# zachramsey/pm-rl

Measured on AMD Instinct MI355X. Metric: env-steps/sec (whole node) at 65k envs x 30 assets; reward MAE vs CPU ref, higher is better.
Workload: dtype f64

## Files before the change

pm-rl_amd/csrc/common.h:

```cpp
#pragma once
#include <hip/hip_runtime.h>

#include <math.h>
#include <stdint.h>

#include "../../include/pmenv.h"
#include "step_plan.h"

namespace pmenv_dev {

constexpr uint32_t kRelaySpin = 1024;

typedef float f4 __attribute__((ext_vector_type(4)));
typedef float f4u __attribute__((ext_vector_type(4), aligned(4)));

struct FastDiv {
    uint32_t mul, shift, d;
};

inline FastDiv make_fastdiv(uint32_t d) {
    FastDiv f;
    f.d = d;
    uint32_t s = 0;
    while ((1ull << s) < d) ++s;
// ... 37 lines not shown
    uint32_t halo_wgs, halo_block, halo_qtot;
    uint32_t halo_hs;
    const double* sv_in;
    const int32_t* sk_in;
    const float* sw_in;
    const float* slc_in;
    double* sv_out;
    int32_t* sk_out;
    float* sw_out;
    float* slc_out;
    const float* halo_in;
    float* halo_out;
    uint32_t per4;
    int32_t* seq;
    FastDiv div_wf, div_f, div_w, div_units;
};

struct HostIO {
    const float* close_in;
    float* chan;
    double* value_out;
    uint32_t* done;
    uint32_t seq;
};


__device__ __forceinline__ const float* env_bar(const StepParams& p, int b) {
    const size_t row = (size_t)p.N * (p.F - 1);
    if (!p.day) return p.bar + (size_t)b * row;
    const int32_t d = p.day[b];
// ... 89 lines not shown
```

pm-rl_amd/csrc/env_step.h:

```cpp
#pragma once
#include "common.h"

namespace pmenv_dev {

struct Scratch {
    double* wv;
    double* yv;
    float* wl;
    float* wp;
    float* bar;
    int* ints;
    int wp_off, bar_off;
};

__device__ __forceinline__ Scratch carve(float* lds, int tile_floats, int N, int F) {
    Scratch s;
    s.wv = reinterpret_cast<double*>(lds + tile_floats);
    s.yv = s.wv + N;
    s.wl = reinterpret_cast<float*>(s.yv + N);
    s.wp = s.wl + N;
    s.bar = s.wp + N;
    s.ints = reinterpret_cast<int*>(s.bar + N * (F - 1));
    s.wp_off = tile_floats + 4 * N + N;
    s.bar_off = s.wp_off + N;
// ... 809 lines not shown
    for (int e = 0; e < 4; ++e) {
        const int pos = sd.kk + e;
        const bool in_row = pos < WF;
        const bool lastday = in_row && pos >= WF - F;
        const bool is_w = in_row && f == F - 1;
        const float bsel = pick(sd.bar_nan, __int_as_float(0x7fc00000),
                                pick(f == 0, sd.xb.x, pick(f == 1, sd.xb.y, pick(f == 2, sd.xb.z, sd.xb.w))));
        const bool w_here = shift_w ? lastday : pos == slot_w;
        const float wv = pick(w_here, sd.xwp, pick(shift_w, sh[e], un[e]));
        v[e] = pick(is_w, wv, pick(lastday, bsel, sh[e]));
        f = f == F - 1 ? 0 : f + 1;
    }
    return f4{v[0], v[1], v[2], v[3]};
}

template <typename Side>
__device__ __forceinline__ f4 compose2(const StepParams& p, int kk, int32_t k, const float (&un)[4],
                                       const float (&sh)[4], Side side) {
    constexpr int F = 5;
    const int W = p.W, WF = W * F;
    const bool shift_w = !(p.ring_mode == PMENV_RING_STORAGE && k >= W - 1);
    const int f0 = kk - (int)fdiv((uint32_t)kk, p.div_f) * F;
    float o[4];
#pragma unroll
    for (int e = 0; e < 4; ++e) {
        const int f = f0 + e >= F ? f0 + e - F : f0 + e;
        o[e] = pick(!shift_w & (f == F - 1), un[e], sh[e]);
    }
    const int slot_w = (int)(((uint32_t)(1 + k) - fdiv((uint32_t)(1 + k), p.div_w) * (uint32_t)W) * F + (F - 1));
    if ((kk + 3 >= WF - F) | (!shift_w & ((uint32_t)(slot_w - kk) <= 3u))) {
        f4 xb;
        float xwp;
        side(xb, xwp);
#pragma unroll
        for (int e = 0; e < 4; ++e) {
            const int pos = kk + e;
            const int f = f0 + e >= F ? f0 + e - F : f0 + e;
            const bool in_row = pos < WF;
            const bool lastday = in_row & (pos >= WF - F);
            const float bsel = pick(f == 0, xb.x, pick(f == 1, xb.y, pick(f == 2, xb.z, xb.w)));
            o[e] = pick(lastday & (f < F - 1), bsel, o[e]);
            o[e] = pick((shift_w & lastday & (f == F - 1)) | (!shift_w & in_row & (pos == slot_w)), xwp, o[e]);
        }
    }
    return f4{o[0], o[1], o[2], o[3]};
}

template <int BLOCK, int POL>
__global__ __launch_bounds__(BLOCK) void advance_flat_kernel(StepParams p, uint32_t qtot) {
    constexpr int kAux = POL == 1 ? 2 : POL == 2 ? 3 : 0;
    const int lane = threadIdx.x & 63;
    const uint32_t wbase = __builtin_amdgcn_readfirstlane(blockIdx.x * BLOCK + (threadIdx.x & ~63u));
    if (wbase >= qtot) return;
    const uint32_t nwave = min(64u, qtot - wbase);
    const auto rs_src = make_rsrc(p.obs + (size_t)wbase * 4, nwave * 16u);
    const f4 own = buf_load4<kAux>(rs_src, (uint32_t)lane * 16u);
    const uint32_t qx = wbase + 64u;
// ... 72 lines not shown
            sd[v].xb = sh_side[wave][ri[v]];
            sd[v].xwp = reinterpret_cast<const float*>(&sh_side[wave][4])[ri[v]];
        }
        const f4 n1 = sh4[j + 1], n2 = sh4[j + 2];
        const float sh[4] = {n1.y, n1.z, n1.w, n2.x};
        const float un[4] = {own[v].x, own[v].y, own[v].z, own[v].w};
        if (ABL & 128) buf_store4<kAux>(rd, (uint32_t)j * 16u, f4{sh[0], sh[1], sh[2], sh[3]});
        else buf_store4<kAux>(rd, (uint32_t)j * 16u, flat_compose(p, sd[v], un, sh));
    }
}

template <int BLOCK, int V, int POL, bool OUT>
__device__ __forceinline__ void flat_wg_body_patch(StepParams& p, uint32_t qtot, f4* sh4) {
    constexpr int kAux = POL == 1 ? 2 : POL == 2 ? 3 : 0;
    constexpr int CPW = BLOCK * V, F = 5;
    __shared__ f4 sh_bar[BLOCK];
    __shared__ float sh_wp[BLOCK];
    __shared__ int32_t sh_kc[BLOCK];
    const int tid = threadIdx.x, lane = tid & 63, wave = tid >> 6;
    const uint32_t c0 = blockIdx.x * CPW;
    const uint32_t nblk = min((uint32_t)CPW, qtot - c0);
    const auto rs = make_rsrc(p.obs + (size_t)c0 * 4, nblk * 16u);
    f4 own[V];
#pragma unroll
    for (int v = 0; v < V; ++v) own[v] = buf_load4<kAux>(rs, (uint32_t)(64 * V * wave + 64 * v + lane) * 16u);
    const uint32_t nh = blockIdx.x + 1 < gridDim.x ? min(2u, qtot - c0 - nblk) : 0u;
    const float* hsrc = OUT ? p.obs + (size_t)(c0 + nblk) * 4 : p.halo + (size_t)blockIdx.x * 8;
    const f4 hal = buf_load4<0>(make_rsrc(hsrc, nh * 16u), tid < 2 ? (uint32_t)tid * 16u : 0xFFFFFFF0u);
    __builtin_amdgcn_sched_barrier(0);
    const int N = p.N, W = p.W, WF = W * F;
    const uint32_t per4 = (uint32_t)(N * WF) >> 2;
    const uint32_t b_lo = fdiv(c0, p.div_units);
    const uint32_t g_lo = b_lo * (uint32_t)N + fdiv(4u * (c0 - b_lo * per4), p.div_wf);
    const uint32_t ql = c0 + nblk - 1u;
    const uint32_t b_hi = fdiv(ql, p.div_units);
    const uint32_t g_hi = b_hi * (uint32_t)N + fdiv(4u * (ql - b_hi * per4) + 3u, p.div_wf);
    if ((uint32_t)tid <= g_hi - g_lo) {
        const uint32_t g = g_lo + (uint32_t)tid;
        const uint32_t b = g / (uint32_t)N, n = g - b * (uint32_t)N;
        const float* barb = env_bar(p, (int)b);
        const float nanv = __int_as_float(0x7fc00000);
        sh_bar[tid] = barb ? *reinterpret_cast<const f4*>(barb + (size_t)n * 4) : f4{nanv, nanv, nanv, nanv};
        sh_wp[tid] = p.w_new[g];
        sh_kc[tid] = p.k[b] - 1;
    }
#pragma unroll
    for (int v = 0; v < V; ++v) sh4[64 * V * wave + 64 * v + lane] = own[v];
    if (tid < 2) sh4[CPW + tid] = hal;
    __syncthreads();
    const auto rd = OUT ? make_rsrc(p.obs_out + (size_t)c0 * 4, nblk * 16u) : rs;
#pragma unroll
    for (int v = 0; v < V; ++v) {
        const int j = 64 * V * wave + 64 * v + lane;
        const uint32_t q = min(c0 + (uint32_t)j, qtot - 1u);
        const uint32_t b = fdiv(q, p.div_units);
        const uint32_t j0 = 4u * (q - b * per4);
        const uint32_t row = fdiv(j0, p.div_wf);
        const int kk = (int)(j0 - row * (uint32_t)WF);
        const int t = (int)(b * (uint32_t)N + row - g_lo);
        const f4 n1 = sh4[j + 1], n2 = sh4[j + 2];
        const float sh[4] = {n1.y, n1.z, n1.w, n2.x};
        const float un[4] = {own[v].x, own[v].y, own[v].z, own[v].w};
        const f4 o = compose2(p, kk, sh_kc[t], un, sh, [&](f4& xb, float& xwp) {
            xb = sh_bar[t];
            xwp = sh_wp[t];
        });
        buf_store4<kAux>(rd, (uint32_t)j * 16u, o);
    }
}

template <int BLOCK, int V, int POL, int ABL = 0>
__global__ __launch_bounds__(BLOCK) void advance_flat_inplace_kernel(StepParams p, uint32_t qtot) {
    __shared__ f4 sh4[BLOCK * V + 2];
    if constexpr (ABL == 0) flat_wg_body_patch<BLOCK, V, POL, false>(p, qtot, sh4);
    else flat_wg_body<BLOCK, V, POL, false, ABL>(p, qtot, sh4);
}

template <int BLOCK, int V, int POL>
__global__ __launch_bounds__(BLOCK) void advance_flat_inplace_perelem_kernel(StepParams p, uint32_t qtot) {
    __shared__ f4 sh4[BLOCK * V + 2];
    flat_wg_body<BLOCK, V, POL, false, 0>(p, qtot, sh4);
}
template <int BLOCK, int V, int POL>
// ... 700 lines not shown
```

pm-rl_amd/csrc/handle.h:

```cpp
#pragma once
#include <hip/hip_runtime.h>

#include <stdarg.h>
#include <stdio.h>
#include <stdlib.h>
#include <string.h>

#include "../../include/pmenv.h"
#include "common.h"
#include "step_plan.h"

struct pmenv : pmenv_host::StepPlan {
    pmenv_cfg cfg;
    int device;
    void* state;
    size_t state_bytes;
    bool owns_state;
    double* value;
    double* sa;
    double* sb;
    int32_t* k;
    float* ring;
    float* last_close;
    float* w_new;
// ... 71 lines not shown
    p.ret_mode = c.ret_mode; p.mu_max_iter = c.mu_max_iter;
    p.rows_per_tile = h->rows_per_tile;
    p.tile_floats = h->tile_floats;
    p.unit_rows = h->unit_rows;
    p.units_per_env = h->units_per_env;
    p.init_cash = c.init_cash; p.commission = c.commission; p.scale = c.reward_scale;
    p.rf = c.risk_free_rate; p.eta = c.sharpe_eta; p.mu_tol = c.mu_tol;
    p.value = h->value; p.k = h->k; p.ring = h->ring; p.last_close = h->last_close;
    p.w_new = h->w_new;
    p.sa = h->sa; p.sb = h->sb;
    p.nonfinite = h->nonfinite;
    p.div_wf = make_fastdiv((uint32_t)(c.window * c.features));
    p.div_f = make_fastdiv((uint32_t)c.features);
    p.div_w = make_fastdiv((uint32_t)c.window);
    p.div_units = make_fastdiv((uint32_t)(h->units_per_env > 0 ? h->units_per_env : 1));
    return p;
}

inline bool aligned4(const void* ptr) { return ((uintptr_t)ptr & 3u) == 0; }

inline int device_cus() {
    static const int cus = [] {
        int dev = 0, n = 0;
        if (hipGetDevice(&dev) != hipSuccess ||
            hipDeviceGetAttribute(&n, hipDeviceAttributeMultiprocessorCount, dev) != hipSuccess || n <= 0)
            n = 256;
        return n;
    }();
    return cus;
}
// ... 47 lines not shown
```

pm-rl_amd/csrc/step_flat.h:

```cpp
#pragma once
#include "scalar_vec.h"

namespace pmenv_dev {

__device__ __forceinline__ ScalarIn scalar_load_snap(const StepParams& p, int b, int lane) {
    const int N = p.N;
    const uint32_t nb = (uint32_t)N * 4u, off = (uint32_t)lane * 4u;
    ScalarIn in;
    in.k = p.sk_in[b];
    in.v_prev = p.sv_in[b];
    in.sa = p.sa[b];
    in.sb = p.sb[b];
    in.a = buf_load1(make_rsrc(p.action + (size_t)b * N, nb), off);
    in.wlf = buf_load1(make_rsrc(p.sw_in + (size_t)b * N, p.commission > 0.0 ? nb : 0u), off);
    in.pl = buf_load1(make_rsrc((p.prices ? p.prices : p.slc_in) + (size_t)b * N, nb), off);
    const float* barb = env_bar(p, b);
    in.bar = buf_load4(make_rsrc(barb ? barb : p.bar, barb ? nb * 4u : 0u), off * 4u);
    in.bar_ok = barb != nullptr;
    in.cn = 0.0f;
    return in;
}

template <int V>
struct FlatTile {
// ... 14 lines not shown
    t.ne = (int)(fdiv(t.c0 + t.nblk - 1u, p.div_units) - t.e_lo) + 1;
    if (wave < t.ne) t.sin = scalar_load_snap(p, (int)t.e_lo + wave, lane);
    __builtin_amdgcn_sched_barrier(0);
    const auto rs = make_rsrc(p.obs + (size_t)t.c0 * 4, t.nblk * 16u);
#pragma unroll
    for (int v = 0; v < V; ++v) t.own[v] = buf_load4<AUX>(rs, (uint32_t)(64 * V * wave + 64 * v + lane) * 16u);
    const uint32_t ntiles = (qtot + CPW - 1) / CPW;
    const uint32_t nh = tile + 1 < ntiles ? min(2u, qtot - t.c0 - t.nblk) : 0u;
    const float* hsrc = OUT ? p.obs + (size_t)(t.c0 + t.nblk) * 4 : p.halo_in + (size_t)tile * 8;
    t.hal = buf_load4<0>(make_rsrc(hsrc, nh * 16u), tid < 2 ? (uint32_t)tid * 16u : 0xFFFFFFF0u);
    __builtin_amdgcn_sched_barrier(0);
}

template <int BLOCK, int V, int AUX, bool OUT>
__device__ __forceinline__ void flat1_process(const StepParams& p, uint32_t qtot, uint32_t tile, const FlatTile<V>& t,
                                              f4* sh4, f4 (*sh_bar)[64], float (*sh_wp)[64], int32_t* sh_k) {
    constexpr int CPW = BLOCK * V, F = 5;
    const int tid = threadIdx.x, lane = tid & 63, wave = __builtin_amdgcn_readfirstlane(tid >> 6);
    const uint32_t per4 = p.per4;
    ScalarMid mid;
    if (wave < t.ne) {
        mid = scalar_core<64, true>(p, (int)t.e_lo + wave, lane, t.sin);
        sh_wp[wave][lane] = mid.wp;
        sh_bar[wave][lane] = t.sin.bar_ok ? t.sin.bar : f4{NAN, NAN, NAN, NAN};
        if (lane == 0) sh_k[wave] = mid.k;
    }
#pragma unroll
    for (int v = 0; v < V; ++v) sh4[64 * V * wave + 64 * v + lane] = t.own[v];
    if (tid < 2) sh4[CPW + tid] = t.hal;
    __syncthreads();
    const int WF = p.W * F;
    const auto rd = make_rsrc((OUT ? p.obs_out : p.obs) + (size_t)t.c0 * 4, t.nblk * 16u);
    const bool first_out = !OUT && tile > 0;
#pragma unroll
    for (int v = 0; v < V; ++v) {
        const int j = 64 * V * wave + 64 * v + lane;
        const uint32_t q = min(t.c0 + (uint32_t)j, qtot - 1u);
        const uint32_t e = fdiv(q, p.div_units);
        const int le = (int)(e - t.e_lo);
        const uint32_t j0 = 4u * (q - e * per4);
        const uint32_t row = fdiv(j0, p.div_wf);
        const int kk = (int)(j0 - row * (uint32_t)WF);
        const f4 n1 = sh4[j + 1], n2 = sh4[j + 2];
        const float sh[4] = {n1.y, n1.z, n1.w, n2.x};
        const float un[4] = {t.own[v].x, t.own[v].y, t.own[v].z, t.own[v].w};
        const f4 o = compose2(p, kk, sh_k[le], un, sh, [&](f4& xb, float& xwp) {
            xb = sh_bar[le][row];
            xwp = sh_wp[le][row];
        });
        buf_store4<AUX>(rd, (uint32_t)j * 16u, o);
        if (first_out && j < 2) reinterpret_cast<f4*>(p.halo_out)[2 * (tile - 1) + j] = o;
    }
    if (wave < t.ne) {
        const int b = (int)t.e_lo + wave;
        const bool owner = (uint64_t)b * per4 >= t.c0;
        scalar_tail<64, true>(p, b, lane, t.sin, mid, owner);
    }
}

template <bool OUT>
__device__ __forceinline__ void flat_seq_enter(StepParams& p) {
    if (!p.seq) return;
    const int c = __builtin_amdgcn_readfirstlane(p.seq[1]);
    if (c) {
        const double* v = p.sv_in; p.sv_in = p.sv_out; p.sv_out = const_cast<double*>(v);
        const int32_t* k = p.sk_in; p.sk_in = p.sk_out; p.sk_out = const_cast<int32_t*>(k);
        const float* w = p.sw_in; p.sw_in = p.sw_out; p.sw_out = const_cast<float*>(w);
// ... 2 lines not shown
    }
    if (blockIdx.x == 0 && threadIdx.x == 0) {
        const uint64_t hobs = OUT ? 0ull : (uint64_t)(uintptr_t)p.obs;
        p.seq[0] = 1 - c;
        p.seq[2] = 1;
        p.seq[4] = (int32_t)(uint32_t)hobs;
        p.seq[5] = (int32_t)(uint32_t)(hobs >> 32);
    }
}

template <int BLOCK, int V, int POL, bool OUT>
__global__ __launch_bounds__(BLOCK) __attribute__((amdgpu_num_sgpr(80))) void step_flat_kernel(StepParams p,
                                                                                              uint32_t qtot) {
    constexpr int CPW = BLOCK * V, WAVES = BLOCK / 64, AUX = POL == 1 ? 2 : 0;
    __shared__ f4 sh4[CPW + 2];
    __shared__ f4 sh_bar[WAVES][64];
    __shared__ float sh_wp[WAVES][64];
    __shared__ int32_t sh_k[WAVES];
    flat_seq_enter<OUT>(p);
    FlatTile<V> t;
    flat1_load<BLOCK, V, AUX, OUT>(p, qtot, blockIdx.x, t);
    flat1_process<BLOCK, V, AUX, OUT>(p, qtot, blockIdx.x, t, sh4, sh_bar, sh_wp, sh_k);
}

template <int A, int BLOCK, int V, int POL, bool OUT>
__global__ __launch_bounds__(BLOCK) void step_flat_vec_kernel(StepParams p, uint32_t qtot) {
    constexpr int kAuxL = POL == 1 ? 2 : 0, kAuxS = POL == 1 ? 2 : 0;
    constexpr int CPW = BLOCK * V, WAVES = BLOCK / 64, F = 5;
    __shared__ f4 sh4[CPW + 2];
    __shared__ f4 sh_bar[WAVES][64];
    __shared__ float sh_wp[WAVES][64];
    __shared__ int32_t sh_k[WAVES], sh_rlo[WAVES];
    const uint32_t tile = blockIdx.x;
    flat_seq_enter<OUT>(p);
    const int tid = threadIdx.x, lane = tid & 63, wave = __builtin_amdgcn_readfirstlane(tid >> 6);
    const int N = p.N, WF = p.W * F;
    const uint32_t per4 = p.per4;
    const uint32_t c0 = tile * (uint32_t)CPW;
    const uint32_t nblk = min((uint32_t)CPW, qtot - c0);
    const uint32_t e_lo = fdiv(c0, p.div_units);
    const int ne = (int)(fdiv(c0 + nblk - 1u, p.div_units) - e_lo) + 1;
    VecIn<A> vin;
    f4 brow = f4{0.f, 0.f, 0.f, 0.f};
    int rlo = 0;
    bool bar_ok = false;
    const int b = (int)e_lo + wave;
    if (wave < ne) {
// ... 8 lines not shown
        const auto rb = make_rsrc(barb ? barb : p.bar, barb ? (uint32_t)(rhi + 1) * 16u : 0u);
        brow = buf_load4<0>(rb, (uint32_t)(rlo + lane) * 16u);
    }
    __builtin_amdgcn_sched_barrier(0);
    const auto rs = make_rsrc(p.obs + (size_t)c0 * 4, nblk * 16u);
    f4 own[V];
#pragma unroll
    for (int v = 0; v < V; ++v) own[v] = buf_load4<kAuxL>(rs, (uint32_t)(64 * V * wave + 64 * v + lane) * 16u);
    const uint32_t ntiles = (qtot + CPW - 1) / CPW;
    const uint32_t nh = tile + 1 < ntiles ? min(2u, qtot - c0 - nblk) : 0u;
    const float* hsrc = OUT ? p.obs + (size_t)(c0 + nblk) * 4 : p.halo_in + (size_t)tile * 8;
    const f4 hal = buf_load4<0>(make_rsrc(hsrc, nh * 16u), tid < 2 ? (uint32_t)tid * 16u : 0xFFFFFFF0u);
    __builtin_amdgcn_sched_barrier(0);
    if (wave < ne) {
        const VecMid<A> mid = vec_core<64, A, true>(p, b, lane, vin);
#pragma unroll
        for (int e = 0; e < A; ++e) {
            const int n = lane + 64 * e;
            if ((unsigned)(n - rlo) < 64u) sh_wp[wave][n - rlo] = mid.wp[e];
        }
        sh_bar[wave][lane] = bar_ok ? brow : f4{NAN, NAN, NAN, NAN};
        if (lane == 0) {
            sh_k[wave] = vin.k;
            sh_rlo[wave] = rlo;
        }
        const bool owner = (uint64_t)b * per4 >= c0;
        vec_tail<64, A, true, true>(p, b, lane, vin, mid, owner);
    }
#pragma unroll
    for (int v = 0; v < V; ++v) sh4[64 * V * wave + 64 * v + lane] = own[v];
    if (tid < 2) sh4[CPW + tid] = hal;
    __syncthreads();
    const auto rd = make_rsrc((OUT ? p.obs_out : p.obs) + (size_t)c0 * 4, nblk * 16u);
    const bool first_out = !OUT && tile > 0;
#pragma unroll
    for (int v = 0; v < V; ++v) {
        const int j = 64 * V * wave + 64 * v + lane;
        const uint32_t q = min(c0 + (uint32_t)j, qtot - 1u);
        const uint32_t e = fdiv(q, p.div_units);
        const int le = (int)(e - e_lo);
        const uint32_t j0 = 4u * (q - e * per4);
        const uint32_t row = fdiv(j0, p.div_wf);
        const int kk = (int)(j0 - row * (uint32_t)WF);
        const f4 n1 = sh4[j + 1], n2 = sh4[j + 2];
        const float sh[4] = {n1.y, n1.z, n1.w, n2.x};
        const float un[4] = {own[v].x, own[v].y, own[v].z, own[v].w};
        const f4 o = compose2(p, kk, sh_k[le], un, sh, [&](f4& xb, float& xwp) {
            const int r = (int)row - sh_rlo[le];
            xb = sh_bar[le][r];
            xwp = sh_wp[le][r];
        });
        buf_store4<kAuxS>(rd, (uint32_t)j * 16u, o);
        if (first_out && j < 2) reinterpret_cast<f4*>(p.halo_out)[2 * (tile - 1) + j] = o;
    }
}

__device__ __forceinline__ void flat_prime(const StepParams& p, bool snap) {
    copy_halo(p);
    if (!snap) return;
    const uint32_t nthr = gridDim.x * blockDim.x;
    const uint32_t tid = blockIdx.x * blockDim.x + threadIdx.x;
    const size_t BN = (size_t)p.B * p.N;
    for (size_t i = tid; i < (size_t)p.B; i += nthr) {
        p.sv_out[i] = p.value[i];
        p.sk_out[i] = p.k[i];
    }
    for (size_t i = tid; i < BN; i += nthr) {
        p.sw_out[i] = p.w_new[i];
        p.slc_out[i] = p.last_close[i];
// ... 27 lines not shown
```

pm-rl_amd/csrc/step_plan.h:

```cpp
#pragma once

#include <stdarg.h>
#include <stdint.h>
#include <stdio.h>

#include "../../include/pmenv.h"

namespace pmenv_dev {

constexpr int kWideMaxAssets = 512;
constexpr int kBlock = 256;
constexpr int kMaxVec = 8;
constexpr int kTileFloats = kBlock * kMaxVec * 4;
constexpr int kScalarWaves = 4;
constexpr int kStreamBlock = 512;

inline size_t scratch_bytes(int tile_floats, int N, int F) {
    return (size_t)tile_floats * 4 + (size_t)N * 16 + (size_t)N * 8 + (size_t)N * (F - 1) * 4 + 16;
}

}

namespace pmenv_host {

constexpr int PMENV_FUSE_DB = 1, PMENV_FUSE_INPLACE = 2;
constexpr int kOneV = 4;
constexpr int kK1Str = 100000;

struct StepPlan {
    int small_block, small_e;
    bool tiny;
    bool surf_stream;
    size_t surf_lds;
// ... 417 lines not shown
```

pm-rl_amd/csrc/step_relay.h:

```cpp
#pragma once
#include "env_step.h"
#include "scalar_vec.h"

namespace pmenv_dev {

struct RelayParams {
    uint32_t scal;
    uint32_t epoch;
    uint64_t* w;
    uint64_t* list;
    uint32_t* done;
    uint32_t spin;
    uint32_t rot;
    uint32_t grid;
    const int32_t* kp_in;
    int32_t* kp_out;
    const float* halo_in;
    float* halo_out;
    uint32_t* seq;
    int32_t* kp;
    float* halo;
    uint32_t B;
    uint32_t halo_stride;
    const float* obs;
// ... 106 lines not shown
            if (env_ok && n < N) relay_put(r.w + (size_t)b * N + n, epoch, __float_as_uint(m.wp[e]));
        }
        if (env_ok && j == 0) kp_out[b] = in.k + 1;
        listed = relay_list_read(r, epoch);
        ts[1] = relay_clock<ST>(listed);
        vec_tail<KL, KA, true>(p, b, lane, in, m);
    }
    ts[2] = relay_clock<ST, true>(0);
    relay_stamps_put<ST>((uint32_t)s, epoch, ts);
    return listed;
}

template <int BLOCK, int V, int POL, bool OUT, bool ADOPT, bool ST = false>
__device__ __forceinline__ bool relay_tile(const StepParams& p, const RelayParams& r, uint32_t qtot, uint32_t spin, uint32_t t,
                                           uint32_t epoch, const int32_t* kp_in, const float* halo_in,
                                           float* halo_out, f4* sh4, f4* sh_bar, float* sh_wp, int32_t* sh_kc,
                                           int32_t* sh_ok, uint64_t t_entry = 0) {
    uint64_t ts[6] = {t_entry, 0, 0, 0, 0, 0};
    constexpr int kAux = POL == 1 ? 2 : 0;
    constexpr int CPW = BLOCK * V, F = 5;
    const int tid = threadIdx.x, lane = tid & 63, wave = tid >> 6;
    const uint32_t c0 = t * CPW;
    const uint32_t nblk = min((uint32_t)CPW, qtot - c0);
    const auto rs = make_rsrc(p.obs + (size_t)c0 * 4, nblk * 16u);
    f4 own[V];
#pragma unroll
    for (int v = 0; v < V; ++v) own[v] = buf_load4<kAux>(rs, (uint32_t)(64 * V * wave + 64 * v + lane) * 16u);
    const uint32_t ntiles = (qtot + CPW - 1) / CPW;
    const uint32_t nh = t + 1 < ntiles ? min(2u, qtot - c0 - nblk) : 0u;
    const float* hsrc = OUT ? p.obs + (size_t)(c0 + nblk) * 4 : halo_in + (size_t)t * 8;
    const f4 hal = buf_load4<0>(make_rsrc(hsrc, nh * 16u), tid < 2 ? (uint32_t)tid * 16u : 0xFFFFFFF0u);
// ... 16 lines not shown
    if (barb) xb = *reinterpret_cast<const f4*>(barb + (size_t)n * 4);
    kc = kp_in[b];
    ww = relay_get(r.w + g);
    bool ready = !mine || (uint32_t)(ww >> 32) == epoch;
    ts[1] = relay_clock<ST>((uint32_t)ww);
    for (uint32_t polls = 0; !ADOPT && !__all(ready) && polls < spin; ++polls) {
        __builtin_amdgcn_s_sleep(2);
        if (!ready) {
            ww = relay_get(r.w + g);
            ready = (uint32_t)(ww >> 32) == epoch;
        }
    }
    const bool wave_ok = __all(ready);
    ts[2] = relay_clock<ST>((uint32_t)ww);
    if (mine) {
        sh_bar[tid] = xb;
        sh_wp[tid] = __uint_as_float((uint32_t)ww);
        sh_kc[tid] = kc;
    }
#pragma unroll
    for (int v = 0; v < V; ++v) sh4[64 * V * wave + 64 * v + lane] = own[v];
    if (tid < 2) sh4[CPW + tid] = hal;
    if (lane == 0) sh_ok[wave] = wave_ok ? 1 : 0;
    __syncthreads();
    ts[3] = relay_clock<ST>(0);
    if constexpr (ADOPT) {
        bool tile_ok = true;
#pragma unroll
        for (int w = 0; w < BLOCK / 64; ++w) tile_ok = tile_ok && sh_ok[w] != 0;
        if (!tile_ok) return false;
        if (tid == 0)
            sh_ok[BLOCK / 64] = __hip_atomic_exchange(r.done + t, epoch, __ATOMIC_RELAXED, __HIP_MEMORY_SCOPE_AGENT) != epoch;
        __syncthreads();
        if (!sh_ok[BLOCK / 64]) return true;
    }
    const auto rd = OUT ? make_rsrc(p.obs_out + (size_t)c0 * 4, nblk * 16u) : rs;
    const bool first_out = !OUT && t > 0;
    bool ok = true;
#pragma unroll
    for (int v = 0; v < V; ++v) {
        const int j = 64 * V * wave + 64 * v + lane;
        const uint32_t q = min(c0 + (uint32_t)j, qtot - 1u);
        const uint32_t bq = fdiv(q, p.div_units);
        const uint32_t j0 = 4u * (q - bq * per4);
        const uint32_t row = fdiv(j0, p.div_wf);
        const int kk = (int)(j0 - row * (uint32_t)WF);
        const int i = (int)(bq * (uint32_t)N + row - g_lo);
        const f4 n1 = sh4[j + 1], n2 = sh4[j + 2];
        const float sh[4] = {n1.y, n1.z, n1.w, n2.x};
        const float un[4] = {own[v].x, own[v].y, own[v].z, own[v].w};
        f4 o = compose2(p, kk, sh_kc[i], un, sh, [&](f4& x, float& xwp) {
            x = sh_bar[i];
            xwp = sh_wp[i];
        });
        if (!ADOPT && v == 0) {
            int32_t okv = 1;
#pragma unroll
            for (int w = 0; w < BLOCK / 64; ++w) okv &= sh_ok[w];
            ok = __builtin_amdgcn_readfirstlane(okv) != 0;
        }
        buf_store4<kAux>(rd, ok ? (uint32_t)j * 16u : 0x80000000u, o);
        if (ok && first_out && j < 2) reinterpret_cast<f4*>(halo_out)[2 * (t - 1) + j] = o;
    }
    ts[4] = relay_clock<ST>(0);
    ts[5] = relay_clock<ST, true>(0);
    relay_stamps_put<ST>(r.scal + t, epoch, ts);
    return ok;
}

template <int BLOCK, int V, int POL, bool OUT, bool SEQ>
__device__ __forceinline__ void relay_adopt(f4* sh4, f4* sh_bar, float* sh_wp, int32_t* sh_kc, int32_t* sh_ok,
                                            uint32_t listed) {
    constexpr int kB = BLOCK / 64 + 1;
    const int wave = threadIdx.x >> 6;
    if ((threadIdx.x & 63) == 0) sh_ok[wave] = (int32_t)__builtin_amdgcn_readfirstlane(listed);
    __syncthreads();
    uint32_t n = 0;
#pragma unroll
    for (int w = 0; w < BLOCK / 64; ++w) n = max(n, (uint32_t)sh_ok[w]);
    if (n == 0) return;
    const KArgs ka = kargs();
    const RelayCtx c = relay_ctx<SEQ>(ka.r);
    for (uint32_t i = 0; i < n; ++i) {
        __syncthreads();
        if (threadIdx.x == 0) {
            const uint64_t e = relay_get(ka.r.list + 1 + i);
            int32_t t = (uint32_t)(e >> 32) == c.epoch ? (int32_t)(uint32_t)e : -1;
            if (t >= 0 && __hip_atomic_load(ka.r.done + t, __ATOMIC_RELAXED, __HIP_MEMORY_SCOPE_AGENT) == c.epoch)
                t = -1;
            sh_ok[kB] = t;
        }
        __syncthreads();
        const int32_t t = __builtin_amdgcn_readfirstlane(sh_ok[kB]);
        if (t >= 0)
            (void)relay_tile<BLOCK, V, POL, OUT, true>(ka.p, ka.r, ka.qtot, 0u, (uint32_t)t, c.epoch, c.kp_in, c.halo_in,
                                                       c.halo_out, sh4, sh_bar, sh_wp, sh_kc, sh_ok);
    }
}

template <int BLOCK, int V, int POL, bool OUT, bool SEQ>
__device__ __forceinline__ void relay_defer(uint32_t t, f4* sh4, f4* sh_bar, float* sh_wp, int32_t* sh_kc,
                                            int32_t* sh_ok) {
    const KArgs ka = kargs();
    const RelayCtx c = relay_ctx<SEQ>(ka.r);
    if (threadIdx.x == 0) {
        uint64_t lw = relay_get(ka.r.list), nw;
        do {
            nw = (uint32_t)(lw >> 32) == c.epoch ? lw + 1 : ((uint64_t)c.epoch << 32) | 1u;
        } while (!__hip_atomic_compare_exchange_strong(ka.r.list, &lw, nw, __ATOMIC_RELAXED, __ATOMIC_RELAXED,
                                                        __HIP_MEMORY_SCOPE_AGENT));
        const uint32_t slot = (uint32_t)(lw >> 32) == c.epoch ? (uint32_t)lw : 0u;
        relay_put(ka.r.list + 1 + slot, c.epoch, t);
        __atomic_signal_fence(__ATOMIC_SEQ_CST);
        __builtin_amdgcn_s_waitcnt(0);
        __atomic_signal_fence(__ATOMIC_SEQ_CST);
    }
    __syncthreads();
    (void)relay_tile<BLOCK, V, POL, OUT, true>(ka.p, ka.r, ka.qtot, 0u, t, c.epoch, c.kp_in, c.halo_in, c.halo_out, sh4,
                                               sh_bar, sh_wp, sh_kc, sh_ok);
}

template <int BLOCK, int V, int POL, bool OUT, int KL, int KA, int OCC = 1, bool SEQ = false, int ANY = 0>
__global__ __launch_bounds__(BLOCK) __attribute__((amdgpu_waves_per_eu(OCC))) void step_relay_kernel(
    StepParams p, RelayParams r, uint32_t qtot) {
    __shared__ f4 sh4[BLOCK * V + 2];
    __shared__ f4 sh_bar[BLOCK];
    __shared__ float sh_wp[BLOCK];
    __shared__ int32_t sh_kc[BLOCK];
    __shared__ int32_t sh_ok[BLOCK / 64 + 2];
    const RelayCtx c = relay_ctx<SEQ>(r);
    if constexpr (SEQ) {
        if (blockIdx.x == 0 && threadIdx.x == 0) {
            const uint64_t hobs = OUT ? 0ull : (uint64_t)(uintptr_t)r.obs;
            r.seq[kSeqD] = (uint32_t)((c.kp_in - r.kp) / r.B) ^ 1u;
            r.seq[kSeqE] = c.epoch;
            r.seq[kSeqV] = 1u;
            r.seq[kSeqHobs] = (uint32_t)hobs;
            r.seq[kSeqHobs + 1] = (uint32_t)(hobs >> 32);
        }
    }
    constexpr bool kSt = ANY == 2;
    const uint64_t t_entry = relay_clock<kSt>(0);
    uint32_t bid = blockIdx.x;
    if constexpr (ANY == 1) {
        bid += r.rot;
        if (bid >= r.grid) bid -= r.grid;
    }
    if (bid < r.scal) {
        const uint32_t listed = relay_scalar<BLOCK, KL, KA, kSt>(p, r, (int)bid, c.epoch, c.kp_out, t_entry);
        relay_adopt<BLOCK, V, POL, OUT, SEQ>(sh4, sh_bar, sh_wp, sh_kc, sh_ok, listed);
    } else if (!relay_tile<BLOCK, V, POL, OUT, false, kSt>(p, r, qtot, ANY == 1 ? r.spin : kRelaySpin, bid - r.scal, c.epoch,
                                                           c.kp_in, c.halo_in, c.halo_out, sh4, sh_bar, sh_wp, sh_kc,
                                                           sh_ok, t_entry)) {
        relay_defer<BLOCK, V, POL, OUT, SEQ>(bid - r.scal, sh4, sh_bar, sh_wp, sh_kc, sh_ok);
    }
}

static __global__ __launch_bounds__(256) void relay_prime_kernel(StepParams p, RelayParams r, int prime_kp, int seq) {
    uint32_t d = r.par;
    bool kp = prime_kp != 0, halo = p.halo != nullptr;
    if (seq) {
        d = __builtin_amdgcn_readfirstlane(r.seq[kSeqD]);
        const uint32_t e = __builtin_amdgcn_readfirstlane(r.seq[kSeqE]);
        const uint32_t v = __builtin_amdgcn_readfirstlane(r.seq[kSeqV]);
        const uint64_t hobs = (uint64_t)__builtin_amdgcn_readfirstlane(r.seq[kSeqHobs]) |
                              ((uint64_t)__builtin_amdgcn_readfirstlane(r.seq[kSeqHobs + 1]) << 32);
        kp = v == 0;
        halo = halo && (v == 0 || hobs != (uint64_t)(uintptr_t)p.obs);
        if (blockIdx.x == 0 && threadIdx.x == 0) {
// ... 16 lines not shown
```

Baseline: 104.1 million.

## Stage last-day bar/weight in packed LDS rows and walk chunk positions incrementally

The per-element fast divisions that map a 4-float chunk to (env,row,kk,f0) are now done once per thread, then advanced by a precomputed constant stride for the remaining unrolled iterations when the plan allows. The last-day bar values and new weight are staged as contiguous 5-float rows in LDS, and the ring slot position is precomputed per row. This lets compose2 fill the patch with simple offset loads instead of nested per-feature selects. The intent is fewer integer ops and selects in the observation-write loop. The cost is a second template instantiation of each loop and some extra clamping logic.

Result: no change. 103.7 million (-0.4%).

```diff
diff --git a/pm-rl_amd/csrc/common.h b/pm-rl_amd/csrc/common.h
--- a/pm-rl_amd/csrc/common.h
+++ b/pm-rl_amd/csrc/common.h
@@ -75,6 +75,7 @@
     uint32_t per4;
     int32_t* seq;
     FastDiv div_wf, div_f, div_w, div_units;
+    ChunkStep cstep;
 };
 
 struct HostIO {
diff --git a/pm-rl_amd/csrc/env_step.h b/pm-rl_amd/csrc/env_step.h
--- a/pm-rl_amd/csrc/env_step.h
+++ b/pm-rl_amd/csrc/env_step.h
@@ -847,33 +847,65 @@
     return f4{v[0], v[1], v[2], v[3]};
 }
 
-template <typename Side>
-__device__ __forceinline__ f4 compose2(const StepParams& p, int kk, int32_t k, const float (&un)[4],
-                                       const float (&sh)[4], Side side) {
+__device__ __forceinline__ ChunkPos chunk_pos_div(const StepParams& p, uint32_t q, uint32_t per4) {
     constexpr int F = 5;
-    const int W = p.W, WF = W * F;
-    const bool shift_w = !(p.ring_mode == PMENV_RING_STORAGE && k >= W - 1);
-    const int f0 = kk - (int)fdiv((uint32_t)kk, p.div_f) * F;
+    ChunkPos c;
+    c.env = fdiv(q, p.div_units);
+    const uint32_t j0 = 4u * (q - c.env * per4);
+    const uint32_t row = fdiv(j0, p.div_wf);
+    c.row = (int)row;
+    c.kk = (int)(j0 - row * (uint32_t)(p.W * F));
+    c.f0 = c.kk - (int)fdiv((uint32_t)c.kk, p.div_f) * F;
+    c.grow = c.env * (uint32_t)p.N + row;
+    return c;
+}
+template <bool ADV>
+__device__ __forceinline__ void chunk_pos_walk(const StepParams& p, ChunkPos& c, bool first, uint32_t q, uint32_t per4) {
+    if (first || !ADV) c = chunk_pos_div(p, q, per4);
+    else chunk_pos_step(c, p.cstep, p.N, p.W * 5, 5);
+}
+template <bool ADV>
+struct ChunkWalk {
+    static constexpr bool adv = ADV;
+};
+template <typename Body>
+__device__ __forceinline__ void chunk_walk_forms(const StepParams& p, Body body) {
+    if (p.cstep.ok) body(ChunkWalk<true>{});
+    else body(ChunkWalk<false>{});
+}
+
+constexpr int kLastPad = 4;
+constexpr int last_floats(int rows) { return 2 * kLastPad + 5 * rows; }
+__device__ __forceinline__ void last_stage(float* last, int r, const f4& bar, float wp) {
+    float* l = last + kLastPad + 5 * r;
+    l[0] = bar.x; l[1] = bar.y; l[2] = bar.z; l[3] = bar.w; l[4] = wp;
+}
+__device__ __forceinline__ int slot_pos(const StepParams& p, int32_t k) {
+    constexpr int F = 5;
+    const bool shift_w = !(p.ring_mode == PMENV_RING_STORAGE && k >= p.W - 1);
+    const int slot_w = (int)(((uint32_t)(1 + k) - fdiv((uint32_t)(1 + k), p.div_w) * (uint32_t)p.W) * F + (F - 1));
+    return shift_w ? -1 : slot_w;
+}
+
+__device__ __forceinline__ f4 compose2(int WF, int kk, int f0, int slot, const float (&un)[4], const float (&sh)[4],
+                                       const float* lastp) {
+    constexpr int F = 5;
+    const int ew = slot >= 0 ? F - 1 - f0 : -1;
     float o[4];
 #pragma unroll
-    for (int e = 0; e < 4; ++e) {
-        const int f = f0 + e >= F ? f0 + e - F : f0 + e;
-        o[e] = pick(!shift_w & (f == F - 1), un[e], sh[e]);
-    }
-    const int slot_w = (int)(((uint32_t)(1 + k) - fdiv((uint32_t)(1 + k), p.div_w) * (uint32_t)W) * F + (F - 1));
-    if ((kk + 3 >= WF - F) | (!shift_w & ((uint32_t)(slot_w - kk) <= 3u))) {
-        f4 xb;
-        float xwp;
-        side(xb, xwp);
+    for (int e = 0; e < 4; ++e) o[e] = e == ew ? un[e] : sh[e];
+    const int d = kk - (WF - F), se = slot - kk;
+    if ((d >= -3) | ((uint32_t)se <= 3u)) {
+        const float* lp = lastp + max(d, -3);
+        float l[4];
+#pragma unroll
+        for (int e = 0; e < 4; ++e) l[e] = lp[e];
+        const float wp = lastp[F - 1];
+        const uint32_t span = slot >= 0 ? F - 1 : F;
 #pragma unroll
         for (int e = 0; e < 4; ++e) {
-            const int pos = kk + e;
-            const int f = f0 + e >= F ? f0 + e - F : f0 + e;
-            const bool in_row = pos < WF;
-            const bool lastday = in_row & (pos >= WF - F);
-            const float bsel = pick(f == 0, xb.x, pick(f == 1, xb.y, pick(f == 2, xb.z, xb.w)));
-            o[e] = pick(lastday & (f < F - 1), bsel, o[e]);
-            o[e] = pick((shift_w & lastday & (f == F - 1)) | (!shift_w & in_row & (pos == slot_w)), xwp, o[e]);
+            o[e] = (uint32_t)(d + e) < span ? l[e] : o[e];
+            o[e] = e == se ? wp : o[e];
         }
     }
     return f4{o[0], o[1], o[2], o[3]};
@@ -976,9 +1008,8 @@
 __device__ __forceinline__ void flat_wg_body_patch(StepParams& p, uint32_t qtot, f4* sh4) {
     constexpr int kAux = POL == 1 ? 2 : POL == 2 ? 3 : 0;
     constexpr int CPW = BLOCK * V, F = 5;
-    __shared__ f4 sh_bar[BLOCK];
-    __shared__ float sh_wp[BLOCK];
-    __shared__ int32_t sh_kc[BLOCK];
+    __shared__ float sh_last[last_floats(BLOCK)];
+    __shared__ int32_t sh_sl[BLOCK];
     const int tid = threadIdx.x, lane = tid & 63, wave = tid >> 6;
     const uint32_t c0 = blockIdx.x * CPW;
     const uint32_t nblk = min((uint32_t)CPW, qtot - c0);
@@ -1002,33 +1033,29 @@
         const uint32_t b = g / (uint32_t)N, n = g - b * (uint32_t)N;
         const float* barb = env_bar(p, (int)b);
         const float nanv = __int_as_float(0x7fc00000);
-        sh_bar[tid] = barb ? *reinterpret_cast<const f4*>(barb + (size_t)n * 4) : f4{nanv, nanv, nanv, nanv};
-        sh_wp[tid] = p.w_new[g];
-        sh_kc[tid] = p.k[b] - 1;
+        last_stage(sh_last, tid, barb ? *reinterpret_cast<const f4*>(barb + (size_t)n * 4) : f4{nanv, nanv, nanv, nanv},
+                   p.w_new[g]);
+        sh_sl[tid] = slot_pos(p, p.k[b] - 1);
     }
 #pragma unroll
     for (int v = 0; v < V; ++v) sh4[64 * V * wave + 64 * v + lane] = own[v];
     if (tid < 2) sh4[CPW + tid] = hal;
     __syncthreads();
     const auto rd = OUT ? make_rsrc(p.obs_out + (size_t)c0 * 4, nblk * 16u) : rs;
-#pragma unroll
-    for (int v = 0; v < V; ++v) {
-        const int j = 64 * V * wave + 64 * v + lane;
-        const uint32_t q = min(c0 + (uint32_t)j, qtot - 1u);
-        const uint32_t b = fdiv(q, p.div_units);
-        const uint32_t j0 = 4u * (q - b * per4);
-        const uint32_t row = fdiv(j0, p.div_wf);
-        const int kk = (int)(j0 - row * (uint32_t)WF);
-        const int t = (int)(b * (uint32_t)N + row - g_lo);
-        const f4 n1 = sh4[j + 1], n2 = sh4[j + 2];
-        const float sh[4] = {n1.y, n1.z, n1.w, n2.x};
-        const float un[4] = {own[v].x, own[v].y, own[v].z, own[v].w};
-        const f4 o = compose2(p, kk, sh_kc[t], un, sh, [&](f4& xb, float& xwp) {
-            xb = sh_bar[t];
-            xwp = sh_wp[t];
-        });
-        buf_store4<kAux>(rd, (uint32_t)j * 16u, o);
-    }
+    chunk_walk_forms(p, [&](auto walk) {
+        ChunkPos cp;
+#pragma unroll
+        for (int v = 0; v < V; ++v) {
+            const int j = 64 * V * wave + 64 * v + lane;
+            chunk_pos_walk<walk.adv>(p, cp, v == 0, min(c0 + (uint32_t)j, qtot - 1u), per4);
+            const int t = (int)min(cp.grow - g_lo, (uint32_t)(BLOCK - 1));
+            const f4 n1 = sh4[j + 1], n2 = sh4[j + 2];
+            const float sh[4] = {n1.y, n1.z, n1.w, n2.x};
+            const float un[4] = {own[v].x, own[v].y, own[v].z, own[v].w};
+            const f4 o = compose2(WF, cp.kk, cp.f0, sh_sl[t], un, sh, sh_last + kLastPad + 5 * t);
+            buf_store4<kAux>(rd, (uint32_t)j * 16u, o);
+        }
+    });
 }
 
 template <int BLOCK, int V, int POL, int ABL = 0>
diff --git a/pm-rl_amd/csrc/handle.h b/pm-rl_amd/csrc/handle.h
--- a/pm-rl_amd/csrc/handle.h
+++ b/pm-rl_amd/csrc/handle.h
@@ -109,6 +109,7 @@
     p.div_f = make_fastdiv((uint32_t)c.features);
     p.div_w = make_fastdiv((uint32_t)c.window);
     p.div_units = make_fastdiv((uint32_t)(h->units_per_env > 0 ? h->units_per_env : 1));
+    p.cstep = pmenv_dev::plan_chunk_step(c.num_assets, c.window, c.features);
     return p;
 }
 
diff --git a/pm-rl_amd/csrc/step_flat.h b/pm-rl_amd/csrc/step_flat.h
--- a/pm-rl_amd/csrc/step_flat.h
+++ b/pm-rl_amd/csrc/step_flat.h
@@ -52,16 +52,16 @@
 
 template <int BLOCK, int V, int AUX, bool OUT>
 __device__ __forceinline__ void flat1_process(const StepParams& p, uint32_t qtot, uint32_t tile, const FlatTile<V>& t,
-                                              f4* sh4, f4 (*sh_bar)[64], float (*sh_wp)[64], int32_t* sh_k) {
-    constexpr int CPW = BLOCK * V, F = 5;
+                                              f4* sh4, float* sh_last, int32_t* sh_sl) {
+    constexpr int CPW = BLOCK * V, WAVES = BLOCK / 64, F = 5;
     const int tid = threadIdx.x, lane = tid & 63, wave = __builtin_amdgcn_readfirstlane(tid >> 6);
     const uint32_t per4 = p.per4;
     ScalarMid mid;
     if (wave < t.ne) {
         mid = scalar_core<64, true>(p, (int)t.e_lo + wave, lane, t.sin);
-        sh_wp[wave][lane] = mid.wp;
-        sh_bar[wave][lane] = t.sin.bar_ok ? t.sin.bar : f4{NAN, NAN, NAN, NAN};
-        if (lane == 0) sh_k[wave] = mid.k;
+        last_stage(sh_last, 64 * wave + lane, t.sin.bar_ok ? t.sin.bar : f4{NAN, NAN, NAN, NAN},
+                   mid.wp);
+        if (lane == 0) sh_sl[wave] = slot_pos(p, mid.k);
     }
 #pragma unroll
     for (int v = 0; v < V; ++v) sh4[64 * V * wave + 64 * v + lane] = t.own[v];
@@ -70,25 +70,21 @@
     const int WF = p.W * F;
     const auto rd = make_rsrc((OUT ? p.obs_out : p.obs) + (size_t)t.c0 * 4, t.nblk * 16u);
     const bool first_out = !OUT && tile > 0;
-#pragma unroll
-    for (int v = 0; v < V; ++v) {
-        const int j = 64 * V * wave + 64 * v + lane;
-        const uint32_t q = min(t.c0 + (uint32_t)j, qtot - 1u);
-        const uint32_t e = fdiv(q, p.div_units);
-        const int le = (int)(e - t.e_lo);
-        const uint32_t j0 = 4u * (q - e * per4);
-        const uint32_t row = fdiv(j0, p.div_wf);
-        const int kk = (int)(j0 - row * (uint32_t)WF);
-        const f4 n1 = sh4[j + 1], n2 = sh4[j + 2];
-        const float sh[4] = {n1.y, n1.z, n1.w, n2.x};
-        const float un[4] = {t.own[v].x, t.own[v].y, t.own[v].z, t.own[v].w};
-        const f4 o = compose2(p, kk, sh_k[le], un, sh, [&](f4& xb, float& xwp) {
-            xb = sh_bar[le][row];
-            xwp = sh_wp[le][row];
-        });
-        buf_store4<AUX>(rd, (uint32_t)j * 16u, o);
-        if (first_out && j < 2) reinterpret_cast<f4*>(p.halo_out)[2 * (tile - 1) + j] = o;
-    }
+    chunk_walk_forms(p, [&](auto walk) {
+        ChunkPos cp;
+    #pragma unroll
+        for (int v = 0; v < V; ++v) {
+            const int j = 64 * V * wave + 64 * v + lane;
+            chunk_pos_walk<walk.adv>(p, cp, v == 0, min(t.c0 + (uint32_t)j, qtot - 1u), per4);
+            const int le = (int)min(cp.env - t.e_lo, (uint32_t)(WAVES - 1));
+            const f4 n1 = sh4[j + 1], n2 = sh4[j + 2];
+            const float sh[4] = {n1.y, n1.z, n1.w, n2.x};
+            const float un[4] = {t.own[v].x, t.own[v].y, t.own[v].z, t.own[v].w};
+            const f4 o = compose2(WF, cp.kk, cp.f0, sh_sl[le], un, sh, sh_last + kLastPad + 5 * (64 * le + cp.row));
+            buf_store4<AUX>(rd, (uint32_t)j * 16u, o);
+            if (first_out && j < 2) reinterpret_cast<f4*>(p.halo_out)[2 * (tile - 1) + j] = o;
+        }
+    });
     if (wave < t.ne) {
         const int b = (int)t.e_lo + wave;
         const bool owner = (uint64_t)b * per4 >= t.c0;
@@ -121,13 +117,12 @@
                                                                                               uint32_t qtot) {
     constexpr int CPW = BLOCK * V, WAVES = BLOCK / 64, AUX = POL == 1 ? 2 : 0;
     __shared__ f4 sh4[CPW + 2];
-    __shared__ f4 sh_bar[WAVES][64];
-    __shared__ float sh_wp[WAVES][64];
-    __shared__ int32_t sh_k[WAVES];
+    __shared__ float sh_last[last_floats(64 * WAVES)];
+    __shared__ int32_t sh_sl[WAVES];
     flat_seq_enter<OUT>(p);
     FlatTile<V> t;
     flat1_load<BLOCK, V, AUX, OUT>(p, qtot, blockIdx.x, t);
-    flat1_process<BLOCK, V, AUX, OUT>(p, qtot, blockIdx.x, t, sh4, sh_bar, sh_wp, sh_k);
+    flat1_process<BLOCK, V, AUX, OUT>(p, qtot, blockIdx.x, t, sh4, sh_last, sh_sl);
 }
 
 template <int A, int BLOCK, int V, int POL, bool OUT>
@@ -135,9 +130,8 @@
     constexpr int kAuxL = POL == 1 ? 2 : 0, kAuxS = POL == 1 ? 2 : 0;
     constexpr int CPW = BLOCK * V, WAVES = BLOCK / 64, F = 5;
     __shared__ f4 sh4[CPW + 2];
-    __shared__ f4 sh_bar[WAVES][64];
-    __shared__ float sh_wp[WAVES][64];
-    __shared__ int32_t sh_k[WAVES], sh_rlo[WAVES];
+    __shared__ float sh_last[last_floats(64 * WAVES)];
+    __shared__ int32_t sh_sl[WAVES], sh_rlo[WAVES];
     const uint32_t tile = blockIdx.x;
     flat_seq_enter<OUT>(p);
     const int tid = threadIdx.x, lane = tid & 63, wave = __builtin_amdgcn_readfirstlane(tid >> 6);
@@ -176,14 +170,16 @@
     __builtin_amdgcn_sched_barrier(0);
     if (wave < ne) {
         const VecMid<A> mid = vec_core<64, A, true>(p, b, lane, vin);
+        float* last = sh_last + kLastPad + 5 * 64 * wave;
 #pragma unroll
         for (int e = 0; e < A; ++e) {
             const int n = lane + 64 * e;
-            if ((unsigned)(n - rlo) < 64u) sh_wp[wave][n - rlo] = mid.wp[e];
-        }
-        sh_bar[wave][lane] = bar_ok ? brow : f4{NAN, NAN, NAN, NAN};
+            if ((unsigned)(n - rlo) < 64u) last[5 * (n - rlo) + 4] = mid.wp[e];
+        }
+        const f4 bx = bar_ok ? brow : f4{NAN, NAN, NAN, NAN};
+        last[5 * lane] = bx.x; last[5 * lane + 1] = bx.y; last[5 * lane + 2] = bx.z; last[5 * lane + 3] = bx.w;
         if (lane == 0) {
-            sh_k[wave] = vin.k;
+            sh_sl[wave] = slot_pos(p, vin.k);
             sh_rlo[wave] = rlo;
         }
         const bool owner = (uint64_t)b * per4 >= c0;
@@ -195,26 +191,22 @@
     __syncthreads();
     const auto rd = make_rsrc((OUT ? p.obs_out : p.obs) + (size_t)c0 * 4, nblk * 16u);
     const bool first_out = !OUT && tile > 0;
-#pragma unroll
-    for (int v = 0; v < V; ++v) {
-        const int j = 64 * V * wave + 64 * v + lane;
-        const uint32_t q = min(c0 + (uint32_t)j, qtot - 1u);
-        const uint32_t e = fdiv(q, p.div_units);
-        const int le = (int)(e - e_lo);
-        const uint32_t j0 = 4u * (q - e * per4);
-        const uint32_t row = fdiv(j0, p.div_wf);
-        const int kk = (int)(j0 - row * (uint32_t)WF);
-        const f4 n1 = sh4[j + 1], n2 = sh4[j + 2];
-        const float sh[4] = {n1.y, n1.z, n1.w, n2.x};
-        const float un[4] = {own[v].x, own[v].y, own[v].z, own[v].w};
-        const f4 o = compose2(p, kk, sh_k[le], un, sh, [&](f4& xb, float& xwp) {
-            const int r = (int)row - sh_rlo[le];
-            xb = sh_bar[le][r];
-            xwp = sh_wp[le][r];
-        });
-        buf_store4<kAuxS>(rd, (uint32_t)j * 16u, o);
-        if (first_out && j < 2) reinterpret_cast<f4*>(p.halo_out)[2 * (tile - 1) + j] = o;
-    }
+    chunk_walk_forms(p, [&](auto walk) {
+        ChunkPos cp;
+    #pragma unroll
+        for (int v = 0; v < V; ++v) {
+            const int j = 64 * V * wave + 64 * v + lane;
+            chunk_pos_walk<walk.adv>(p, cp, v == 0, min(c0 + (uint32_t)j, qtot - 1u), per4);
+            const int le = (int)min(cp.env - e_lo, (uint32_t)(WAVES - 1));
+            const int r = (cp.row - sh_rlo[le]) & 63;
+            const f4 n1 = sh4[j + 1], n2 = sh4[j + 2];
+            const float sh[4] = {n1.y, n1.z, n1.w, n2.x};
+            const float un[4] = {own[v].x, own[v].y, own[v].z, own[v].w};
+            const f4 o = compose2(WF, cp.kk, cp.f0, sh_sl[le], un, sh, sh_last + kLastPad + 5 * (64 * le + r));
+            buf_store4<kAuxS>(rd, (uint32_t)j * 16u, o);
+            if (first_out && j < 2) reinterpret_cast<f4*>(p.halo_out)[2 * (tile - 1) + j] = o;
+        }
+    });
 }
 
 __device__ __forceinline__ void flat_prime(const StepParams& p, bool snap) {
diff --git a/pm-rl_amd/csrc/step_plan.h b/pm-rl_amd/csrc/step_plan.h
--- a/pm-rl_amd/csrc/step_plan.h
+++ b/pm-rl_amd/csrc/step_plan.h
@@ -17,6 +17,44 @@
 
 inline size_t scratch_bytes(int tile_floats, int N, int F) {
     return (size_t)tile_floats * 4 + (size_t)N * 16 + (size_t)N * 8 + (size_t)N * (F - 1) * 4 + 16;
+}
+
+
+constexpr int kChunkStride = 256;
+
+struct ChunkStep {
+    int32_t rows, kk;
+    int32_t ok;
+};
+
+struct ChunkPos {
+    uint32_t env;
+    uint32_t grow;
+    int32_t row, kk, f0;
+};
+
+inline ChunkStep plan_chunk_step(int N, int W, int F) {
+    ChunkStep s;
+    const int WF = W * F;
+    s.rows = kChunkStride / WF;
+    s.kk = kChunkStride % WF;
+    s.ok = F == 5 && WF >= 4 && s.rows + (s.kk >= 4 ? 1 : 0) <= N;
+    return s;
+}
+
+constexpr void chunk_pos_step(ChunkPos& c, const ChunkStep& s, int N, int WF, int F) {
+    int32_t kk = c.kk + s.kk, dr = s.rows;
+    if (kk >= WF) { kk -= WF; dr += 1; }
+    int32_t row = c.row + dr;
+    uint32_t env = c.env;
+    if (row >= N) { row -= N; env += 1u; }
+    int32_t f0 = c.f0 + kChunkStride % F;
+    if (f0 >= F) f0 -= F;
+    c.kk = kk;
+    c.row = row;
+    c.env = env;
+    c.grow += (uint32_t)dr;
+    c.f0 = f0;
 }
 
 }
diff --git a/pm-rl_amd/csrc/step_relay.h b/pm-rl_amd/csrc/step_relay.h
--- a/pm-rl_amd/csrc/step_relay.h
+++ b/pm-rl_amd/csrc/step_relay.h
@@ -144,7 +144,7 @@
 template <int BLOCK, int V, int POL, bool OUT, bool ADOPT, bool ST = false>
 __device__ __forceinline__ bool relay_tile(const StepParams& p, const RelayParams& r, uint32_t qtot, uint32_t spin, uint32_t t,
                                            uint32_t epoch, const int32_t* kp_in, const float* halo_in,
-                                           float* halo_out, f4* sh4, f4* sh_bar, float* sh_wp, int32_t* sh_kc,
+                                           float* halo_out, f4* sh4, float* sh_last, int32_t* sh_sl,
                                            int32_t* sh_ok, uint64_t t_entry = 0) {
     uint64_t ts[6] = {t_entry, 0, 0, 0, 0, 0};
     constexpr int kAux = POL == 1 ? 2 : 0;
@@ -191,9 +191,8 @@
     const bool wave_ok = __all(ready);
     ts[2] = relay_clock<ST>((uint32_t)ww);
     if (mine) {
-        sh_bar[tid] = xb;
-        sh_wp[tid] = __uint_as_float((uint32_t)ww);
-        sh_kc[tid] = kc;
+        last_stage(sh_last, tid, xb, __uint_as_float((uint32_t)ww));
+        sh_sl[tid] = slot_pos(p, kc);
     }
 #pragma unroll
     for (int v = 0; v < V; ++v) sh4[64 * V * wave + 64 * v + lane] = own[v];
@@ -214,31 +213,27 @@
     const auto rd = OUT ? make_rsrc(p.obs_out + (size_t)c0 * 4, nblk * 16u) : rs;
     const bool first_out = !OUT && t > 0;
     bool ok = true;
-#pragma unroll
-    for (int v = 0; v < V; ++v) {
-        const int j = 64 * V * wave + 64 * v + lane;
-        const uint32_t q = min(c0 + (uint32_t)j, qtot - 1u);
-        const uint32_t bq = fdiv(q, p.div_units);
-        const uint32_t j0 = 4u * (q - bq * per4);
-        const uint32_t row = fdiv(j0, p.div_wf);
-        const int kk = (int)(j0 - row * (uint32_t)WF);
-        const int i = (int)(bq * (uint32_t)N + row - g_lo);
-        const f4 n1 = sh4[j + 1], n2 = sh4[j + 2];
-        const float sh[4] = {n1.y, n1.z, n1.w, n2.x};
-        const float un[4] = {own[v].x, own[v].y, own[v].z, own[v].w};
-        f4 o = compose2(p, kk, sh_kc[i], un, sh, [&](f4& x, float& xwp) {
-            x = sh_bar[i];
-            xwp = sh_wp[i];
-        });
-        if (!ADOPT && v == 0) {
-            int32_t okv = 1;
-#pragma unroll
-            for (int w = 0; w < BLOCK / 64; ++w) okv &= sh_ok[w];
-            ok = __builtin_amdgcn_readfirstlane(okv) != 0;
-        }
-        buf_store4<kAux>(rd, ok ? (uint32_t)j * 16u : 0x80000000u, o);
-        if (ok && first_out && j < 2) reinterpret_cast<f4*>(halo_out)[2 * (t - 1) + j] = o;
-    }
+    chunk_walk_forms(p, [&](auto walk) {
+        ChunkPos cp;
+    #pragma unroll
+        for (int v = 0; v < V; ++v) {
+            const int j = 64 * V * wave + 64 * v + lane;
+            chunk_pos_walk<walk.adv>(p, cp, v == 0, min(c0 + (uint32_t)j, qtot - 1u), per4);
+            const int i = (int)min(cp.grow - g_lo, (uint32_t)(BLOCK - 1));
+            const f4 n1 = sh4[j + 1], n2 = sh4[j + 2];
+            const float sh[4] = {n1.y, n1.z, n1.w, n2.x};
+            const float un[4] = {own[v].x, own[v].y, own[v].z, own[v].w};
+            f4 o = compose2(WF, cp.kk, cp.f0, sh_sl[i], un, sh, sh_last + kLastPad + 5 * i);
+            if (!ADOPT && v == 0) {
+                int32_t okv = 1;
+    #pragma unroll
+                for (int w = 0; w < BLOCK / 64; ++w) okv &= sh_ok[w];
+                ok = __builtin_amdgcn_readfirstlane(okv) != 0;
+            }
+            buf_store4<kAux>(rd, ok ? (uint32_t)j * 16u : 0x80000000u, o);
+            if (ok && first_out && j < 2) reinterpret_cast<f4*>(halo_out)[2 * (t - 1) + j] = o;
+        }
+    });
     ts[4] = relay_clock<ST>(0);
     ts[5] = relay_clock<ST, true>(0);
     relay_stamps_put<ST>(r.scal + t, epoch, ts);
@@ -246,8 +241,7 @@
 }
 
 template <int BLOCK, int V, int POL, bool OUT, bool SEQ>
-__device__ __forceinline__ void relay_adopt(f4* sh4, f4* sh_bar, float* sh_wp, int32_t* sh_kc, int32_t* sh_ok,
-                                            uint32_t listed) {
+__device__ __forceinline__ void relay_adopt(f4* sh4, float* sh_last, int32_t* sh_sl, int32_t* sh_ok, uint32_t listed) {
     constexpr int kB = BLOCK / 64 + 1;
     const int wave = threadIdx.x >> 6;
     if ((threadIdx.x & 63) == 0) sh_ok[wave] = (int32_t)__builtin_amdgcn_readfirstlane(listed);
@@ -271,13 +265,12 @@
         const int32_t t = __builtin_amdgcn_readfirstlane(sh_ok[kB]);
         if (t >= 0)
             (void)relay_tile<BLOCK, V, POL, OUT, true>(ka.p, ka.r, ka.qtot, 0u, (uint32_t)t, c.epoch, c.kp_in, c.halo_in,
-                                                       c.halo_out, sh4, sh_bar, sh_wp, sh_kc, sh_ok);
+                                                       c.halo_out, sh4, sh_last, sh_sl, sh_ok);
     }
 }
 
 template <int BLOCK, int V, int POL, bool OUT, bool SEQ>
-__device__ __forceinline__ void relay_defer(uint32_t t, f4* sh4, f4* sh_bar, float* sh_wp, int32_t* sh_kc,
-                                            int32_t* sh_ok) {
+__device__ __forceinline__ void relay_defer(uint32_t t, f4* sh4, float* sh_last, int32_t* sh_sl, int32_t* sh_ok) {
     const KArgs ka = kargs();
     const RelayCtx c = relay_ctx<SEQ>(ka.r);
     if (threadIdx.x == 0) {
@@ -294,16 +287,15 @@
     }
     __syncthreads();
     (void)relay_tile<BLOCK, V, POL, OUT, true>(ka.p, ka.r, ka.qtot, 0u, t, c.epoch, c.kp_in, c.halo_in, c.halo_out, sh4,
-                                               sh_bar, sh_wp, sh_kc, sh_ok);
+                                               sh_last, sh_sl, sh_ok);
 }
 
 template <int BLOCK, int V, int POL, bool OUT, int KL, int KA, int OCC = 1, bool SEQ = false, int ANY = 0>
 __global__ __launch_bounds__(BLOCK) __attribute__((amdgpu_waves_per_eu(OCC))) void step_relay_kernel(
     StepParams p, RelayParams r, uint32_t qtot) {
     __shared__ f4 sh4[BLOCK * V + 2];
-    __shared__ f4 sh_bar[BLOCK];
-    __shared__ float sh_wp[BLOCK];
-    __shared__ int32_t sh_kc[BLOCK];
+    __shared__ float sh_last[last_floats(BLOCK)];
+    __shared__ int32_t sh_sl[BLOCK];
     __shared__ int32_t sh_ok[BLOCK / 64 + 2];
     const RelayCtx c = relay_ctx<SEQ>(r);
     if constexpr (SEQ) {
@@ -325,11 +317,11 @@
     }
     if (bid < r.scal) {
         const uint32_t listed = relay_scalar<BLOCK, KL, KA, kSt>(p, r, (int)bid, c.epoch, c.kp_out, t_entry);
-        relay_adopt<BLOCK, V, POL, OUT, SEQ>(sh4, sh_bar, sh_wp, sh_kc, sh_ok, listed);
+        relay_adopt<BLOCK, V, POL, OUT, SEQ>(sh4, sh_last, sh_sl, sh_ok, listed);
     } else if (!relay_tile<BLOCK, V, POL, OUT, false, kSt>(p, r, qtot, ANY == 1 ? r.spin : kRelaySpin, bid - r.scal, c.epoch,
-                                                           c.kp_in, c.halo_in, c.halo_out, sh4, sh_bar, sh_wp, sh_kc,
+                                                           c.kp_in, c.halo_in, c.halo_out, sh4, sh_last, sh_sl,
                                                            sh_ok, t_entry)) {
-        relay_defer<BLOCK, V, POL, OUT, SEQ>(bid - r.scal, sh4, sh_bar, sh_wp, sh_kc, sh_ok);
+        relay_defer<BLOCK, V, POL, OUT, SEQ>(bid - r.scal, sh4, sh_last, sh_sl, sh_ok);
     }
 }
 
```
